# mako443/Text2Pos-CVPR2022

Measured on AMD Instinct MI355X. Metric: cells+queries encoded/sec and top-k retrieval QPS, 256-pt cells, 12k-cell DB, higher is better.
Workload: dtype f16x3 (fp32 operands split hi+lo into fp16, 3 f16 MFMAs, fp32 accumulate; fp32-class error) for the encoders / f64 MFMA for the ranking

## Files before the change

text2pos-cvpr2022_amd/csrc/sa3.hip:

```cpp
#include "t2p_common.h"

#ifndef T2P_SA3_ABL
#define T2P_SA3_ABL 0
#endif
#define SB() __builtin_amdgcn_sched_barrier(0)
#define AS4 __attribute__((address_space(4)))

namespace t2p {
namespace {

constexpr int K = 256, N = 256, NC = 32, ND = 64, TR = 32, NW = 8, NT = 64 * NW;
constexpr int LDHH = K + 8;
constexpr int PLANE = TR * LDHH;
constexpr int S16 = K / 16;
constexpr int MAXR = NC * 33;

constexpr int OFF_TILE = 0;
constexpr int OFF_ACC = OFF_TILE + 2 * 2 * PLANE * 2;
constexpr int OFF_BTAB = OFF_ACC + (NC + 1) * N * 4;
constexpr int OFF_WP = OFF_BTAB + (NC + 1) * K * 4;
constexpr int OFF_CPOS = OFF_WP + 3 * K * 4;
constexpr int OFF_BIAS = OFF_CPOS + 512;
constexpr int OFF_DST = OFF_BIAS + N * 4;
constexpr int LDS_BYTES = OFF_DST + 4 * TR * 2;
static_assert(LDS_BYTES <= 160 * 1024, "LDS budget");

#define MFMA32(a, b, c) __builtin_amdgcn_mfma_f32_16x16x32_f16(a, b, c, 0, 0, 0)

template <typename T>
__device__ __forceinline__ const AS4 T* as_const(const T* p) {
    return (const AS4 T*)p;
}
__device__ __forceinline__ void lds_fmax(float* p, float v) {
    (void)__hip_atomic_fetch_max(p, v, __ATOMIC_RELAXED, __HIP_MEMORY_SCOPE_WORKGROUP);
}

struct It {
    int g;
    int r0;
    int n;
    int sb;
};

__global__ __launch_bounds__(NT, 2) void k_sa3(SaParams p) {
    extern __shared__ __attribute__((aligned(16))) char lds[];
    _Float16* const tile = (_Float16*)(lds + OFF_TILE);
    float* const accl = (float*)(lds + OFF_ACC);
    float* const btab = (float*)(lds + OFF_BTAB);
    float* const wpl = (float*)(lds + OFF_WP);
    float* const cposl = (float*)(lds + OFF_CPOS);
    float* const biasl = (float*)(lds + OFF_BIAS);
    uint16_t* const dstl = (uint16_t*)(lds + OFF_DST);

    const int tid = threadIdx.x, lane = tid & 63;
    const int wave = __builtin_amdgcn_readfirstlane(tid >> 6);

    const AS4 uint32_t* const n_rows_c = as_const((const uint32_t*)p.n_rows);
    const AS4 int32_t* const first_c = as_const(p.first);
    const AS4 uint32_t* const rows_c = as_const((const uint32_t*)p.rows);
    const AS4 int32_t* const bounds_c = as_const(p.bounds_ws);

    constexpr int S32 = K / 32;
    const int q16 = lane >> 4, i16 = lane & 15;
    half8 w_hi[2][S32], w_lo[2][S32];
    {
        const uint4* wp = (const uint4*)p.W_x3;
        constexpr int PLANE_U4 = (N / 32) * S16 * 64;
#pragma unroll
        for (int cb = 0; cb < 2; cb++)
#pragma unroll
            for (int s = 0; s < S32; s++) {
                const int k0 = 64 * q16 + 8 * s;
                const int idx = ((wave * S16 + (k0 % (K / 2)) / 8) * 2 + k0 / (K / 2)) * 32 + 16 * cb + i16;
                w_hi[cb][s] = __builtin_bit_cast(half8, wp[idx]);
                w_lo[cb][s] = __builtin_bit_cast(half8, wp[PLANE_U4 + idx]);
            }
    }
    for (int i = tid; i < N; i += NT) biasl[i] = p.bias[i];
    for (int i = tid; i < (NC + 1) * N; i += NT) accl[i] = -__builtin_inff();
    for (int i = tid; i < 3 * K; i += NT) wpl[i] = p.wp[i];
    for (int i = tid; i < K; i += NT) btab[NC * K + i] = 0.f;
    for (int i = tid; i < 4 * TR; i += NT) dstl[i] = (uint16_t)(NC * N * 4);
    int gtop = 0;

    const int g_begin = bounds_c[blockIdx.x], g_end = bounds_c[blockIdx.x + 1];

    auto obj_n = [&](int g) -> int { return g < g_end ? (int)((n_rows_c[g >> 1] >> ((g & 1) * 16)) & 0xFFFFu) : 0; };
    auto obj_sb = [&](int g) -> int {
        if (g >= g_end) return 0;
        const int f = first_c[g];
        return f * ND + (g - f) * NC;
    };
    auto advance = [&](It it) -> It {
        it.r0 += TR;
        if (it.r0 >= it.n) {
            it.g++;
            it.r0 = 0;
            it.n = obj_n(it.g);
            it.sb = obj_sb(it.g);
        }
        return it;
    };
    auto valid = [&](const It& it) { return it.g < g_end; };

    const int c4 = lane;
    float npos = 0.f;
    auto fetch_pos = [&](int g) {
        if (tid < 3 * NC && g < g_end) npos = p.out[((int64_t)g * NC + tid / 3) * (int64_t)p.ldo + N + tid % 3];
    };
    auto build_b = [&](int g) {
        if (tid < 3 * NC) cposl[tid] = npos;
        fetch_pos(g + 1);
        lds_barrier();
        const f32x4 w0 = *(const f32x4*)(wpl + c4 * 4), w1 = *(const f32x4*)(wpl + K + c4 * 4), w2 = *(const f32x4*)(wpl + 2 * K + c4 * 4);
#pragma unroll
        for (int i = 0; i < NC / NW; i++) {
            const int c = wave + NW * i;
            const float px = cposl[3 * c], py = cposl[3 * c + 1], pz = cposl[3 * c + 2];
            f32x4 v;
#pragma unroll
            for (int e = 0; e < 4; e++) {
                float a = px * w0[e];
                a = fmaf(py, w1[e], a);
                a = fmaf(pz, w2[e], a);
                v[e] = a;
            }
            *(f32x4*)(btab + c * K + c4 * 4) = v;
        }
        lds_barrier();
    };
    auto flush = [&](int g) {
        float* o = p.out + (int64_t)g * NC * (int64_t)p.ldo;
        int top = gtop;
        typedef int i32x4 __attribute__((ext_vector_type(4)));
#pragma unroll 2
        for (int i = tid; i < NC * (N / 4); i += NT) {
            const int c = i / (N / 4), col = (i % (N / 4)) * 4;
            const f32x4 raw = *(const f32x4*)(accl + c * N + col);
            const f32x4 bq = *(const f32x4*)(biasl + col);
            f32x4 v;
#pragma unroll
            for (int e = 0; e < 4; e++) {
                const float r = fmaxf(raw[e] + bq[e], 0.f);
                const int bits = __float_as_int(r);
                top = bits > top ? bits : top;
                v[e] = r * p.out_scale;
            }
            *(f32x4*)(o + c * (int64_t)p.ldo + col) = v;
            *(i32x4*)(accl + c * N + col) = i32x4{(int)0xFF800000, (int)0xFF800000, (int)0xFF800000, (int)0xFF800000};
        }
        gtop = top;
    };

    f32x4 sa[4];
    f32x4 bq;
    uint32_t boff[4];
    f32x4 vv;
    fp16x2 vh01, vh23;
    const uint32_t lane16 = (uint32_t)lane * 16u;

    auto load_meta = [&](const It& it) -> uint2 {
        uint2 m{0xFFFFFFFFu, 0xFFFFFFFFu};
        if (valid(it)) {
            const uint32_t e = (uint32_t)it.g * (uint32_t)MAXR + (uint32_t)(it.r0 + 4 * wave);
            m.x = rows_c[e / 2];
            m.y = rows_c[e / 2 + 1];
        }
        return m;
    };
    auto issue = [&](const It& it, const uint2& m, int k, uint32_t& dpack_lo, uint32_t& dpack_hi) {
        const uint32_t word = (k & 2) ? m.y : m.x;
        const uint32_t e16 = (k & 1) ? (word >> 16) : (word & 0xFFFFu);
        const bool pad = !valid(it) || it.r0 + 4 * wave + k >= it.n;
        const uint32_t mm = pad ? 0u : e16;
        const uint32_t src = mm & 0xFFu, d = mm >> 8, dl = pad ? (uint32_t)NC : (d & 127u);
        const uint32_t g = (uint32_t)(valid(it) ? it.g : g_end - 1);
        const uint32_t srow = (d & 0x80u) ? ((uint32_t)it.sb + src) : (g * (uint32_t)ND + src);
        const float* rowp = p.A + (size_t)srow * K;
        if constexpr (T2P_SA3_ABL & 2) {
            const float f = __uint_as_float(((uint32_t)(uintptr_t)rowp & 0xFFFFu) | 0x3f000000u);
            sa[k] = f32x4{f, f, f, f};
        } else
            sa[k] = *(const f32x4*)((const char*)rowp + lane16);
        boff[k] = dl * (uint32_t)(K * 4);
        const uint32_t dv = dl * (uint32_t)(N * 4);
        if (k == 0) dpack_lo = dv;
        else if (k == 1) dpack_lo |= dv << 16;
        else if (k == 2) dpack_hi = dv;
        else dpack_hi |= dv << 16;
    };
    auto load_b = [&](int k) { bq = *(const f32x4*)((const char*)btab + boff[k] + lane16); };
    auto stage_a = [&](int buf, int k) {
        _Float16* dsth = tile + buf * 2 * PLANE;
        uint2 ph;
        if constexpr (T2P_SA3_ABL & 64) {
            ph.x = __float_as_uint(sa[k][0]) ^ __float_as_uint(bq[0]);
            ph.y = __float_as_uint(sa[k][1]) ^ __float_as_uint(bq[1]);
            vv = sa[k];
        } else {
            const f32x4 t = sa[k] - bq;
#pragma unroll
            for (int e = 0; e < 4; e++) vv[e] = fmaxf(t[e], 0.f);
            vh01 = cvt_pk_f16(vv[0], vv[1]);
            vh23 = cvt_pk_f16(vv[2], vv[3]);
            ph.x = __builtin_bit_cast(uint32_t, vh01);
            ph.y = __builtin_bit_cast(uint32_t, vh23);
        }
        if constexpr (T2P_SA3_ABL & 4) asm volatile("" ::"v"(ph.x), "v"(ph.y));
        else *(uint2*)(dsth + (4 * wave + k) * LDHH + c4 * 4) = ph;
    };
    auto stage_b = [&](int buf, int k) {
        _Float16* dsth = tile + buf * 2 * PLANE;
        uint2 pl;
        if constexpr (T2P_SA3_ABL & 64) {
            pl.x = __float_as_uint(vv[2]);
            pl.y = __float_as_uint(vv[3]);
        } else {
            pl.x = split_lo_pk(vh01, vv[0], vv[1]);
            pl.y = split_lo_pk(vh23, vv[2], vv[3]);
        }
        if constexpr (T2P_SA3_ABL & 4) asm volatile("" ::"v"(pl.x), "v"(pl.y));
        else *(uint2*)(dsth + PLANE + (4 * wave + k) * LDHH + c4 * 4) = pl;
    };
    auto put_dst = [&](int slot, uint32_t lo, uint32_t hi) {
        if (lane == 0) *(uint2*)(dstl + slot * TR + 4 * wave) = uint2{lo, hi};
    };

    if (g_begin >= g_end) return;

    It it_c{g_begin, 0, obj_n(g_begin), obj_sb(g_begin)};
    It it_s = advance(it_c);
    It it_g = advance(it_s);
    It it_m = advance(it_g);
    fetch_pos(g_begin);
    uint32_t dlo = 0, dhi = 0;
    {
        const uint2 m0 = load_meta(it_c);
#pragma unroll
        for (int k = 0; k < 4; k++) issue(it_c, m0, k, dlo, dhi);
    }
    __syncthreads();
    put_dst(0, dlo, dhi);
    build_b(g_begin);
#pragma unroll
    for (int k = 0; k < 4; k++) {
        load_b(k);
        stage_a(0, k);
        stage_b(0, k);
    }
    {
        const uint2 m1 = load_meta(it_s);
#pragma unroll
        for (int k = 0; k < 4; k++) issue(it_s, m1, k, dlo, dhi);
        put_dst(1, dlo, dhi);
    }
    uint2 meta_g = load_meta(it_g);
    __syncthreads();

    int flush_g = -1, flush_g1 = -1;
    f32x16 rr[2];
#pragma unroll
    for (int e = 0; e < 16; e++) rr[0][e] = rr[1][e] = -__builtin_inff();
    float* const acc_col = accl + wave * 32 + i16;

    int t = 0;
    int newest = 0;
    for (; valid(it_c);) {
#pragma unroll
        for (int half = 0; half < 2; half++, t++) {
            if (half > 0 && !valid(it_c)) break;
            {
                bool fence = false;
                if (flush_g >= 0 && !(T2P_SA3_ABL & 128)) {
                    flush(flush_g);
                    flush_g = -1;
                    fence = true;
                }
                if (valid(it_s) && it_s.r0 == 0 && !(T2P_SA3_ABL & 128)) {
                    build_b(it_s.g);
                    fence = false;
                }
                if (fence) lds_barrier();
            }
            load_b(0);
            const int buf = half, sbuf = half ^ 1;
            const int dslot = (t + 2) & 3;
            It it_n = it_m;
            f32x16& acc = rr[half ^ 1];
            const f32x16& prev = rr[half];
            uint2 four[2];
            {
                const uint16_t* dl = dstl + ((t + 3) & 3) * TR;
#pragma unroll
                for (int rb = 0; rb < 2; rb++) four[rb] = *(const uint2*)(dl + 16 * rb + 4 * q16);
            }
            const _Float16* hrow = tile + buf * 2 * PLANE + i16 * LDHH + q16 * 64;
            half8 a_hi[2], a_lo[2];
#pragma unroll
            for (int rb = 0; rb < 2; rb++) {
                a_hi[rb] = *(const half8*)(hrow + rb * 16 * LDHH);
                a_lo[rb] = *(const half8*)(hrow + PLANE + rb * 16 * LDHH);
            }
            uint2 meta_m{0xFFFFFFFFu, 0xFFFFFFFFu};
            typedef float f32x4v __attribute__((ext_vector_type(4)));
            const f32x4v kZero4 = {0.f, 0.f, 0.f, 0.f};
            f32x4v blk[4];
#pragma unroll
            for (int sl = 0; sl < 4 * S32; sl++) {
                const int s32 = sl >> 2, b = sl & 3, rb = b >> 1, cb = b & 1;
                SB();
                if (s32 + 1 < S32 && !(T2P_SA3_ABL & 8)) {
                    if (b == 2) {
                        a_hi[0] = *(const half8*)(hrow + (s32 + 1) * 8);
                        a_lo[0] = *(const half8*)(hrow + PLANE + (s32 + 1) * 8);
                    }
                }
                if (s32 > 0 && b == 0 && !(T2P_SA3_ABL & 8)) {
                    a_hi[1] = *(const half8*)(hrow + 16 * LDHH + s32 * 8);
                    a_lo[1] = *(const half8*)(hrow + PLANE + 16 * LDHH + s32 * 8);
                }
                blk[b] = MFMA32(a_hi[rb], w_hi[cb][s32], s32 == 0 ? kZero4 : blk[b]);
                blk[b] = MFMA32(a_hi[rb], w_lo[cb][s32], blk[b]);
                if constexpr (!(T2P_SA3_ABL & 16)) blk[b] = MFMA32(a_lo[rb], w_hi[cb][s32], blk[b]);
                SB();
                {
                    const int w = sl;
                    if (w == 0) meta_m = load_meta(it_m);
#pragma unroll
                    for (int c = (w < 12 ? w : 12); c < (w < 12 ? w + 1 : 12); c++) {
                        const int k = c / 3, part = c % 3;
                        if (part == 0) stage_a(sbuf, k);
                        else if (part == 1) stage_b(sbuf, k);
                        else {
                            issue(it_g, meta_g, k, dlo, dhi);
                            if (k + 1 < 4) load_b(k + 1);
                            else put_dst(dslot, dlo, dhi);
                        }
                    }
                    if (w >= 16) {
                        const int e = w - 16, erb = e >> 3, ecb = (e >> 2) & 1, v = e & 3;
                        const uint32_t pair = (v & 2) ? four[erb].y : four[erb].x;
                        const uint32_t off = (v & 1) ? (pair >> 16) : (pair & 0xFFFFu);
                        if constexpr (T2P_SA3_ABL & 1) asm volatile("" ::"v"(prev[e]), "v"(off));
                        else lds_fmax((float*)((char*)acc_col + off) + 16 * ecb, prev[e]);
                    }
                    if (w == 2 * S32 - 1) it_n = advance(it_m);
                }
            }
#pragma unroll
            for (int b = 0; b < 4; b++)
#pragma unroll
                for (int v = 0; v < 4; v++) acc[8 * (b >> 1) + 4 * (b & 1) + v] = blk[b][v];
            SB();
            const bool obj_done = it_c.r0 + TR >= it_c.n;
            newest = half ^ 1;
            flush_g = flush_g1;
            flush_g1 = obj_done ? it_c.g : -1;
            meta_g = meta_m;
            it_c = it_s;
            it_s = it_g;
            it_g = it_m;
            it_m = it_n;
            if constexpr (!(T2P_SA3_ABL & 32)) __syncthreads();
        }
    }
    if (flush_g >= 0) {
        flush(flush_g);
        lds_barrier();
    }
    {
        const uint16_t* dl = dstl + ((t + 3) & 3) * TR;
        const f32x16& last = rr[newest];
        uint2 four[2];
#pragma unroll
        for (int rb = 0; rb < 2; rb++) four[rb] = *(const uint2*)(dl + 16 * rb + 4 * q16);
#pragma unroll
        for (int e = 0; e < 16; e++) {
            const int erb = e >> 3, ecb = (e >> 2) & 1, v = e & 3;
            const uint32_t pair = (v & 2) ? four[erb].y : four[erb].x;
            const uint32_t off = (v & 1) ? (pair >> 16) : (pair & 0xFFFFu);
            if constexpr (T2P_SA3_ABL & 1) asm volatile("" ::"v"(last[e]), "v"(off));
            else lds_fmax((float*)((char*)acc_col + off) + 16 * ecb, last[e]);
        }
        __syncthreads();
        if (flush_g1 >= 0) flush(flush_g1);
    }
    uint32_t gbits = 0;
    guard_track_bits(gbits, gtop);
    if (p.amax_out != nullptr && lane == 0 && gbits != 0u)
        atomicMax(p.amax_out, __float_as_uint(__uint_as_float(gbits) * p.out_scale));
}

}

bool sa3_selected(int H, int C, const SaParams& p) {
    return H == 256 && C == 256 && p.W_x3 != nullptr && p.wp != nullptr;
}

int sa3_launch_shape(int64_t n_obj, int* tile_rows, int* n_wg) {
    int n = matrix_wgs();
    if (n > 1024) n = 1024;
    if (n > n_obj) n = (int)n_obj;
    *tile_rows = TR;
    *n_wg = n;
    return 0;
}

int launch_sa3(const SaParams& p, hipStream_t st) {
    T2P_CHECK_ARG(p.n_cent == NC && p.n_dense == ND, "sa3: built for %d dense points / %d centroids per object (got %d / %d)", ND, NC,
                  p.n_dense, p.n_cent);
    T2P_CHECK_ARG(p.balanced, "sa3: needs the balanced object ranges of launch_sa_balance_levels");
    T2P_TRY(reserve_lds((const void*)k_sa3, LDS_BYTES, "sa3"));
    if (p.n_obj <= 0) return 0;
    T2P_CHECK_ARG(((uintptr_t)p.out & 15) == 0 && p.ldo % 4 == 0 && ((uintptr_t)p.A & 15) == 0 && ((uintptr_t)p.rows & 7) == 0 &&
                      ((uintptr_t)p.n_rows & 3) == 0,
                  "sa3: tables and output rows must be 16-byte aligned (ldo = %d)", p.ldo);
    T2P_CHECK_ARG(p.n_obj * (int64_t)ND < (1LL << 31), "sa3: chunk too large for 32-bit row indices");
    int tr, n_wg;
    T2P_TRY(sa3_launch_shape(p.n_obj, &tr, &n_wg));
    ProfScope ps_("ws_edge_sa_k256_n256", st);
    T2P_REPEAT(ps_) hipLaunchKernelGGL(k_sa3, dim3(n_wg), dim3(NT), LDS_BYTES, st, p);
    T2P_CHECK_LAUNCH("sa3");
    return 0;
}

}
```

Measured before the change: 159,700.

## Interleave per-wave accumulator drain into the MFMA loop and decouple position staging

Replaces the standalone block-wide flush of finished object accumulators with a per-wave drain split into four slices. Each wave drains only the columns it owns, and the slices are issued inside the MFMA schedule slots, so the flush overlaps compute instead of running as a separate phase with a barrier. Position staging (put_pos) is also split from the B-table build and issued one stage earlier, which removes a barrier from build_b. The risk is more register and scheduling pressure in the hot loop, and correctness now depends on each wave owning its drained columns without cross-wave synchronisation.

```diff
diff --git a/text2pos-cvpr2022_amd/csrc/sa3.hip b/text2pos-cvpr2022_amd/csrc/sa3.hip
--- a/text2pos-cvpr2022_amd/csrc/sa3.hip
+++ b/text2pos-cvpr2022_amd/csrc/sa3.hip
@@ -108,10 +108,11 @@
     auto fetch_pos = [&](int g) {
         if (tid < 3 * NC && g < g_end) npos = p.out[((int64_t)g * NC + tid / 3) * (int64_t)p.ldo + N + tid % 3];
     };
-    auto build_b = [&](int g) {
+    auto put_pos = [&](int g) {
         if (tid < 3 * NC) cposl[tid] = npos;
         fetch_pos(g + 1);
-        lds_barrier();
+    };
+    auto build_b = [&]() {
         const f32x4 w0 = *(const f32x4*)(wpl + c4 * 4), w1 = *(const f32x4*)(wpl + K + c4 * 4), w2 = *(const f32x4*)(wpl + 2 * K + c4 * 4);
 #pragma unroll
         for (int i = 0; i < NC / NW; i++) {
@@ -129,27 +130,26 @@
         }
         lds_barrier();
     };
-    auto flush = [&](int g) {
-        float* o = p.out + (int64_t)g * NC * (int64_t)p.ldo;
+    const uint32_t d_acc = (uint32_t)((lane >> 3) * (N * 4) + wave * 128 + (lane & 7) * 16);
+    const uint32_t d_out = (uint32_t)(((lane >> 3) * p.ldo + wave * 32 + (lane & 7) * 4) * 4);
+    auto drain = [&](int g, int j) {
+        typedef int i32x4 __attribute__((ext_vector_type(4)));
+        char* const a = (char*)accl + d_acc + j * (8 * N * 4);
+        const f32x4 raw = *(const f32x4*)a;
+        const f32x4 bb = *(const f32x4*)((const char*)biasl + wave * 128 + (lane & 7) * 16);
+        float* const o = p.out + ((int64_t)g * NC + 8 * j) * (int64_t)p.ldo;
         int top = gtop;
-        typedef int i32x4 __attribute__((ext_vector_type(4)));
-#pragma unroll 2
-        for (int i = tid; i < NC * (N / 4); i += NT) {
-            const int c = i / (N / 4), col = (i % (N / 4)) * 4;
-            const f32x4 raw = *(const f32x4*)(accl + c * N + col);
-            const f32x4 bq = *(const f32x4*)(biasl + col);
-            f32x4 v;
-#pragma unroll
-            for (int e = 0; e < 4; e++) {
-                const float r = fmaxf(raw[e] + bq[e], 0.f);
-                const int bits = __float_as_int(r);
-                top = bits > top ? bits : top;
-                v[e] = r * p.out_scale;
-            }
-            *(f32x4*)(o + c * (int64_t)p.ldo + col) = v;
-            *(i32x4*)(accl + c * N + col) = i32x4{(int)0xFF800000, (int)0xFF800000, (int)0xFF800000, (int)0xFF800000};
+        f32x4 v;
+#pragma unroll
+        for (int e = 0; e < 4; e++) {
+            const float r = fmaxf(raw[e] + bb[e], 0.f);
+            const int bits = __float_as_int(r);
+            top = bits > top ? bits : top;
+            v[e] = r * p.out_scale;
         }
         gtop = top;
+        *(f32x4*)((char*)o + d_out) = v;
+        *(i32x4*)a = i32x4{(int)0xFF800000, (int)0xFF800000, (int)0xFF800000, (int)0xFF800000};
     };
 
     f32x4 sa[4];
@@ -241,7 +241,10 @@
     }
     __syncthreads();
     put_dst(0, dlo, dhi);
-    build_b(g_begin);
+    put_pos(g_begin);
+    lds_barrier();
+    build_b();
+    if (valid(it_s) && it_s.r0 == 0) put_pos(it_s.g);
 #pragma unroll
     for (int k = 0; k < 4; k++) {
         load_b(k);
@@ -269,18 +272,9 @@
 #pragma unroll
         for (int half = 0; half < 2; half++, t++) {
             if (half > 0 && !valid(it_c)) break;
-            {
-                bool fence = false;
-                if (flush_g >= 0 && !(T2P_SA3_ABL & 128)) {
-                    flush(flush_g);
-                    flush_g = -1;
-                    fence = true;
-                }
-                if (valid(it_s) && it_s.r0 == 0 && !(T2P_SA3_ABL & 128)) {
-                    build_b(it_s.g);
-                    fence = false;
-                }
-                if (fence) lds_barrier();
+            if constexpr (!(T2P_SA3_ABL & 128)) {
+                if (valid(it_s) && it_s.r0 == 0) build_b();
+                if (valid(it_g) && it_g.r0 == 0) put_pos(it_g.g);
             }
             load_b(0);
             const int buf = half, sbuf = half ^ 1;
@@ -344,6 +338,11 @@
                         if constexpr (T2P_SA3_ABL & 1) asm volatile("" ::"v"(prev[e]), "v"(off));
                         else lds_fmax((float*)((char*)acc_col + off) + 16 * ecb, prev[e]);
                     }
+                    if (w >= 12 && w < 16 && !(T2P_SA3_ABL & 128)) {
+                        int fg = flush_g;
+                        asm volatile("" : "+s"(fg));
+                        if (fg >= 0) drain(fg, w - 12);
+                    }
                     if (w == 2 * S32 - 1) it_n = advance(it_m);
                 }
             }
@@ -364,9 +363,9 @@
             if constexpr (!(T2P_SA3_ABL & 32)) __syncthreads();
         }
     }
-    if (flush_g >= 0) {
-        flush(flush_g);
-        lds_barrier();
+    if (flush_g >= 0 && !(T2P_SA3_ABL & 128)) {
+#pragma unroll
+        for (int j = 0; j < 4; j++) drain(flush_g, j);
     }
     {
         const uint16_t* dl = dstl + ((t + 3) & 3) * TR;
@@ -382,8 +381,10 @@
             if constexpr (T2P_SA3_ABL & 1) asm volatile("" ::"v"(last[e]), "v"(off));
             else lds_fmax((float*)((char*)acc_col + off) + 16 * ecb, last[e]);
         }
-        __syncthreads();
-        if (flush_g1 >= 0) flush(flush_g1);
+        if (flush_g1 >= 0 && !(T2P_SA3_ABL & 128)) {
+#pragma unroll
+            for (int j = 0; j < 4; j++) drain(flush_g1, j);
+        }
     }
     uint32_t gbits = 0;
     guard_track_bits(gbits, gtop);
```

After: 160,000, median of 3. No clear change (+0.2%).
